# microsoft/ctsTraffic

Hardware: AMD Instinct MI355X
Metric: GiB/s verified, 64 KiB buffers device-resident; % MI355X HBM roofline (higher is better)
Workload: dtype u8

## Files before the change

ctstraffic_amd/csrc/cts_engine.cpp:

```cpp
#include <hip/hip_runtime_api.h>

#include <algorithm>
#include <atomic>
#include <cctype>
#include <chrono>
#include <condition_variable>
#include <cstdio>
#include <cstdlib>
#include <cstring>
#include <memory>
#include <mutex>
#include <new>
#include <string>
#include <system_error>
#include <thread>
#include <vector>

#include "cts_engine.h"
#include "cts_internal.hpp"
#include "cts_slices.hpp"

struct Mailbox;

struct cts_engine {
// ... 440 lines not shown
    if (parts == nullptr && slots == nullptr) return;
    DeviceQuiesce q(e->device);
    if (parts) (void)hipHostFree(parts);
    if (slots) (void)hipHostFree(slots);
}

const cts::LaunchGeometry& cts::engine_geometry(const cts_engine* e, int* device)
{
    if (device != nullptr) *device = e->device;
    return e->geo;
}

extern "C" {

const char* cts_version(void) { return "ctstraffic_amd 0.3.0 (gfx950)"; }

const char* cts_status_string(int status)
{
    switch (status) {
    case CTS_OK: return "ok";
    case CTS_E_INVALID: return "invalid argument";
    case CTS_E_HIP: return "HIP runtime error";
    case CTS_E_NOMEM: return "out of memory";
    case CTS_E_NO_DEVICE: return "no such HIP device";
    case CTS_E_UNAVAILABLE: return "runtime library unavailable (RCCL)";
    case CTS_E_TIMEOUT: return "timed out (nothing freed; retry)";
    default: return "unknown status";
    }
}

int cts_engine_create(int device, cts_engine** out)
{
    if (out == nullptr) return CTS_E_INVALID;
    *out = nullptr;
    int count = 0;
    if (hipGetDeviceCount(&count) != hipSuccess || count <= 0) return CTS_E_NO_DEVICE;
    if (device < 0 || device >= count) return CTS_E_NO_DEVICE;
    DeviceGuard g(device);
    if (!g.ok) return CTS_E_HIP;
    cts_engine* e = new (std::nothrow) cts_engine();
    if (e == nullptr) return CTS_E_NOMEM;
    e->device = device;
    int cus = 0;
    if (hipDeviceGetAttribute(&cus, hipDeviceAttributeMultiprocessorCount, device) == hipSuccess && cus > 0)
        e->geo.num_cus = cus;
    e->geo.blocks_per_cu = env_int("CTS_BLOCKS_PER_CU", e->geo.blocks_per_cu);
    e->geo.nontemporal = env_int("CTS_NT_LOADS", e->geo.nontemporal);
    e->geo.small_threshold = env_int("CTS_SMALL_THRESHOLD", e->geo.small_threshold);
    e->geo.small_blocks_per_cu = env_int("CTS_SMALL_BLOCKS_PER_CU", e->geo.small_blocks_per_cu);
    e->geo.fill_blocks_per_cu = env_int("CTS_FILL_BLOCKS_PER_CU", e->geo.fill_blocks_per_cu);
    e->geo.small_chunk = env_int("CTS_SMALL_CHUNK", e->geo.small_chunk);
    e->geo.fill_nt = env_int("CTS_FILL_NT", e->geo.fill_nt);
    e->geo.ring_fill_blocks_per_cu = env_int("CTS_RING_FILL_BLOCKS_PER_CU", e->geo.ring_fill_blocks_per_cu);
    e->sync_mailbox = env_int("CTS_SYNC_MAILBOX", e->sync_mailbox) ? 1 : 0;
    if (hipStreamCreateWithFlags(&e->stream, hipStreamNonBlocking) != hipSuccess) {
        delete e;
        return CTS_E_HIP;
    }
    void* p = nullptr;
    if (host_alloc_mapped(cts::kSliceMax * sizeof(cts_buf_desc), &p) != CTS_OK) {
        cts_engine_destroy(e);
        return CTS_E_NOMEM;
    }
    e->stage_desc = static_cast<cts_buf_desc*>(p);
    if (host_alloc_mapped(cts::kSliceMax * sizeof(cts_verify_result), &p) != CTS_OK) {
        cts_engine_destroy(e);
        return CTS_E_NOMEM;
    }
    e->stage_res = static_cast<cts_verify_result*>(p);
    *out = e;
    return CTS_OK;
}

int cts_engine_destroy(cts_engine* e)
{
    if (e == nullptr) return CTS_E_INVALID;
    e->mail.reset();
    {
        DeviceGuard g(e->device);
        if (e->stream) {
            (void)hipStreamSynchronize(e->stream);
            (void)hipStreamDestroy(e->stream);
        }
    }
    {
        DeviceQuiesce q(e->device);
        for (auto& st : e->stage_pool) (void)hipHostFree(st.p);
        e->stage_pool.clear();
        if (e->stage) (void)hipHostFree(e->stage);
        if (e->stage_desc) (void)hipHostFree(e->stage_desc);
        if (e->stage_res) (void)hipHostFree(e->stage_res);
        if (e->batch_desc) (void)hipHostFree(e->batch_desc);
        if (e->batch_res) (void)hipHostFree(e->batch_res);
        if (e->batch_ctr) (void)hipHostFree(e->batch_ctr);
    }
    delete e;
    return CTS_OK;
}

int cts_engine_device(const cts_engine* e) { return e ? e->device : CTS_E_INVALID; }

int cts_engine_numa_node(const cts_engine* e)
{
    if (e == nullptr) return -1;
    char bus[64] = {0};
    if (hipDeviceGetPCIBusId(bus, (int)sizeof(bus), e->device) != hipSuccess) return -1;
// ... 507 lines not shown
```

ctstraffic_amd/csrc/cts_internal.hpp:

```cpp
#pragma once

#include <hip/hip_runtime_api.h>
#include <stdint.h>

#include "cts_connections.h"
#include "cts_engine.h"
#include "cts_media_stream.h"
#include "cts_media_stream_conns.h"

namespace cts {

constexpr int kCounterSlots = 8;
enum CounterSlot {
    kBytesChecked = 0,
    kBytesOk = 1,
    kBuffersChecked = 2,
    kBuffersFailed = 3,
    kMismatchedBytes = 4,
    kConnectionsFailed = 5
};
constexpr int kCounterCount = 6;
static_assert(kCounterCount <= kCounterSlots, "counters fit a shard line");

inline cts_counters_ex counters_ex_of(const uint64_t* v)
{
    return cts_counters_ex{v[kBytesChecked],  v[kBytesOk],         v[kBuffersChecked],
                           v[kBuffersFailed], v[kMismatchedBytes], v[kConnectionsFailed]};
}
inline cts_counters counters_of(const cts_counters_ex& x)
{
    return cts_counters{x.bytes_checked, x.bytes_ok, x.buffers_checked, x.buffers_failed, x.mismatched_bytes};
}

constexpr int kVerifyKernelId = 25;
constexpr int kSmallKernelId = 15;
constexpr int kMediaStreamKernelId = 3;

struct LaunchGeometry {
    int num_cus = 256;
    int blocks_per_cu = 4;
    int small_blocks_per_cu = 64;
    int nontemporal = 1;
    int small_threshold = 8192;
    int small_chunk = 0;
    int fill_nt = 2;
    int fill_blocks_per_cu = 1;
    int ring_fill_blocks_per_cu = 4;
};

struct alignas(64) MailSlot {
    uint64_t ptr_exp;
    uint64_t len_seq;
    uint64_t pad[6];
};
static_assert(sizeof(MailSlot) == 64, "one cache line per slot");
inline void mail_write(MailSlot* s, uint64_t ptr_exp, uint64_t len_seq)
{
    __atomic_store_n(&s->ptr_exp, ptr_exp, __ATOMIC_RELAXED);
    __atomic_store_n(&s->len_seq, len_seq, __ATOMIC_RELEASE);
}
struct alignas(16) MailPart {
    uint64_t g0;
    uint64_t g1;
};
constexpr uint32_t kMailPieceBytes = 4096;
#ifndef CTS_MAIL_GROUP
#define CTS_MAIL_GROUP 4
#endif
constexpr uint32_t kMailGroup = CTS_MAIL_GROUP;
#if defined(__HIP__)
__host__ __device__
#endif
inline uint32_t mail_parts(uint64_t ptr, uint32_t len)
{
    if (len == 0) return kMailGroup;
    const uint64_t pieces = (((ptr & 15u) + (uint64_t)len + 15u) / 16u * 16u + kMailPieceBytes - 1) / kMailPieceBytes;
    return pieces < kMailGroup ? (uint32_t)pieces : kMailGroup;
}
constexpr uint32_t kMailMaxGroups = 64;
constexpr uint32_t kMailSkip = 0xFFFFFFFFu;
struct MailStarts {
    uint64_t j[kMailMaxGroups];
};
hipError_t launch_mailbox(const MailSlot* slots, MailPart* parts, uint32_t per_group, const MailStarts& starts,
                          uint32_t groups, uint64_t idle_ticks, hipStream_t stream, uint64_t delay_ticks = 0);

hipError_t launch_counters_fold(const void* block, uint64_t* out, bool accumulate, hipStream_t stream);

hipError_t launch_verify(const uint8_t* arena, uint64_t arena_bytes, const cts_buf_desc* descs, uint32_t n,
                         uint32_t max_length_hint, cts_verify_result* results, uint64_t* counters,
                         uint32_t* conn_first_fail, uint32_t n_conns, hipStream_t stream,
                         const LaunchGeometry& geo);

hipError_t launch_verify_strided(const uint8_t* arena, uint64_t arena_bytes, uint32_t stride, const uint32_t* lens,
                                 uint32_t n, uint32_t skip_head, uint32_t expected, uint32_t conn_index,
                                 cts_verify_result* results, uint64_t* counters, uint32_t* conn_first_fail,
                                 uint32_t n_conns, hipStream_t stream, const LaunchGeometry& geo);

hipError_t launch_verify_at(const uint8_t* arena, uint64_t arena_bytes, const cts_buf_desc* descs, uint32_t n,
                            uint32_t max_length_hint, cts_verify_result* results, uint64_t* counters,
                            uint32_t* conn_first_fail, uint32_t n_conns, uint32_t base_index, hipStream_t stream,
// ... 80 lines not shown
```

ctstraffic_amd/csrc/cts_kernels.hip:

```cpp
#include <hip/hip_runtime.h>

#include <type_traits>

#include "cts_internal.hpp"

namespace cts {

typedef uint32_t u32x4 __attribute__((ext_vector_type(4)));
constexpr uint32_t kNone = 0xFFFFFFFFu;
constexpr int kBlock = 256;

__device__ __forceinline__ uint32_t pattern_byte_dev(uint32_t pos)
{
    pos &= 0xFFFFu;
    return (pos & 1u) ? (pos >> 9) : ((pos >> 1) & 0xFFu);
}

__device__ __forceinline__ u32x4 expected_chunk(uint32_t q, uint32_t sh)
{
    const uint32_t k = q >> 1;
    const uint32_t base = __umul24(k, 0x10001u) + 0x10000u;
    const uint32_t w0 = base & 0x7FFF7FFFu;
    const uint32_t w1 = (base + 0x20002u) & 0x7FFF7FFFu;
    const uint32_t w2 = (base + 0x40004u) & 0x7FFF7FFFu;
    const uint32_t w3 = (base + 0x60006u) & 0x7FFF7FFFu;
    const uint32_t w4 = (base + 0x80008u) & 0x7FFF7FFFu;
    return u32x4{__builtin_amdgcn_alignbyte(w1, w0, sh), __builtin_amdgcn_alignbyte(w2, w1, sh),
                 __builtin_amdgcn_alignbyte(w3, w2, sh), __builtin_amdgcn_alignbyte(w4, w3, sh)};
}

__device__ __forceinline__ uint32_t nonzero_bytes(uint32_t x)
{
    return (((x & 0x7F7F7F7Fu) + 0x7F7F7F7Fu) | x) & 0x80808080u;
}

__device__ __forceinline__ uint32_t low_bytes_mask(int nb)
{
    return (uint32_t)((1ull << (8 * nb)) - 1ull);
}

__device__ __forceinline__ u32x4 range_mask(uint32_t lo, uint32_t hi)
{
    u32x4 m;
#pragma unroll
    for (int w = 0; w < 4; ++w) {
        int a = (int)lo - 4 * w;
        int b = (int)hi - 4 * w;
        a = a < 0 ? 0 : (a > 4 ? 4 : a);
        b = b < 0 ? 0 : (b > 4 ? 4 : b);
        m[w] = (b > a) ? (low_bytes_mask(b) & ~low_bytes_mask(a)) : 0u;
    }
    return m;
}

// ... 875 lines not shown
    }
    uint64_t v[kCounterCount];
    v[kRefBytesRecv] = wave_sum64(bytes_recv);
    v[kRefBytesOk] = wave_sum64(bytes_ok);
    v[kRefBuffersRecv] = wave_sum(bufs_recv);
    v[kRefBuffersFailed] = wave_sum(bufs_failed);
    v[kRefBytesAfterFailure] = wave_sum64(bytes_after);
    v[kRefBuffersAfterFailure] = wave_sum(bufs_after);
    if ((threadIdx.x & 63u) == 0u) {
#pragma unroll
        for (int k = 0; k < kCounterCount; ++k) red[threadIdx.x / 64][k] = v[k];
    }
    __syncthreads();
    if (threadIdx.x < (unsigned)kCounterCount) {
        uint64_t sum = 0;
#pragma unroll
        for (int w = 0; w < kBlock / 64; ++w) sum += red[w][threadIdx.x];
        if (sum)
            atomicAdd((unsigned long long*)&ref[(blockIdx.x % CTS_COUNTER_SHARDS) * kCounterSlots + threadIdx.x],
                      (unsigned long long)sum);
    }
}


__device__ __forceinline__ void block_add_six(const uint64_t (&v)[kCounterCount], uint64_t (*red)[kCounterCount],
                                              uint64_t* __restrict__ block)
{
    if ((threadIdx.x & 63u) == 0u) {
#pragma unroll
        for (int k = 0; k < kCounterCount; ++k) red[threadIdx.x / 64][k] = v[k];
    }
    __syncthreads();
    if (threadIdx.x < (unsigned)kCounterCount) {
        uint64_t sum = 0;
#pragma unroll
        for (int w = 0; w < kBlock / 64; ++w) sum += red[w][threadIdx.x];
        if (sum)
            atomicAdd((unsigned long long*)&block[(blockIdx.x % CTS_COUNTER_SHARDS) * kCounterSlots + threadIdx.x],
                      (unsigned long long)sum);
    }
}

__device__ __forceinline__ void conn_run_add(cts_conn_state* __restrict__ state, uint32_t conn, uint32_t n_conns,
                                             uint64_t recv, uint64_t after, uint32_t nrecv, uint32_t nafter)
{
    if (conn >= n_conns) return;
    unsigned long long* p = reinterpret_cast<unsigned long long*>(state + conn);
    if (recv) atomicAdd(p + 0, (unsigned long long)recv);
    if (nrecv) atomicAdd(p + 1, (unsigned long long)nrecv);
    if (after) atomicAdd(p + 2, (unsigned long long)after);
    if (nafter) atomicAdd(p + 3, (unsigned long long)nafter);
}

template <bool NT, bool STRIDED>
__global__ void __launch_bounds__(kBlock)
    conn_accumulate(uint64_t arena_bytes, VSource src, uint32_t n, uint32_t base_index,
                    const uint32_t* __restrict__ conn_first_fail, uint32_t n_conns, uint64_t* __restrict__ ref,
                    cts_conn_state* __restrict__ state, uint32_t span)
{
    __shared__ uint64_t red[kBlock / 64][kCounterCount];
    const uint32_t lane = threadIdx.x & 63u;
    const uint64_t lo = ((uint64_t)blockIdx.x * (kBlock / 64) + threadIdx.x / 64) * span;
    const uint64_t hi = lo + span < (uint64_t)n ? lo + span : (uint64_t)n;
    uint64_t bytes_recv = 0, bytes_ok = 0, bytes_after = 0;
    uint32_t bufs_recv = 0, bufs_failed = 0, bufs_after = 0;
    __shared__ uint64_t tail_sum[kBlock / 64][4];
    __shared__ uint32_t tail_key[kBlock / 64][2];
    uint32_t ckey = kNone, cnrecv = 0, cnafter = 0;
    uint64_t crecv = 0, cafter = 0;
    bool whole = true;
    uint64_t pa = 0, pb = 0;
    uint32_t pnrecv = 0, pnafter = 0;
    bool parked = false;
    uint32_t ring_first = kNone;
    if constexpr (STRIDED) ring_first = src.conn_index < n_conns ? conn_first_fail[src.conn_index] : kNone;
    cts_buf_desc dn = cts_buf_desc{0, 0, 65536u, 0, 0};
    if (lo < hi) dn = refview_desc<NT, STRIDED>(src, lo + lane < hi ? lo + lane : hi - 1);
    for (uint64_t t = lo; t < hi; t += 64) {
        const uint64_t i = t + lane;
        const cts_buf_desc d = dn;
        if (t + 64 < hi) dn = refview_desc<NT, STRIDED>(src, i + 64 < hi ? i + 64 : hi - 1);
        const bool ok = i < hi && !desc_bad(d, arena_bytes);
        const uint32_t key = ok ? d.conn_index : kNone;
        const uint32_t first = STRIDED ? ring_first : (key < n_conns ? conn_first_fail[key] : kNone);
        const uint32_t g = base_index + (uint32_t)i;
        const uint32_t vlen = ok ? d.length - d.skip_head : 0u;
        const bool recv = ok && g <= first, after = ok && g > first;
        if (recv) {
            bytes_recv += vlen;
            bufs_recv += 1u;
            if (g < first) bytes_ok += vlen;
            else bufs_failed += 1u;
        } else if (after) {
            bytes_after += vlen;
            bufs_after += 1u;
        }
        const uint32_t below = (uint32_t)__shfl_up((int)key, 1, 64);
        const bool head = lane == 0u || key != below;
        const uint64_t heads = __ballot(head);
        const uint32_t h = 63u - (uint32_t)__builtin_clzll(heads & (~0ull >> (63u - lane)));
        const bool merge = (uint32_t)__shfl((int)key, 0, 64) == ckey;
        if (heads == 1ull && merge) {
            pa += recv ? vlen : 0u;
            pb += after ? vlen : 0u;
            pnrecv += recv ? 1u : 0u;
            pnafter += after ? 1u : 0u;
            parked = true;
            continue;
        }
        if (parked) {
            crecv += wave_sum64(pa);
            cafter += wave_sum64(pb);
            cnrecv += wave_sum(pnrecv);
            cnafter += wave_sum(pnafter);
            pa = pb = 0;
            pnrecv = pnafter = 0;
            parked = false;
        }
        uint64_t a = recv ? vlen : 0u, b = after ? vlen : 0u;
        uint32_t c = (recv ? 1u : 0u) | (after ? 0x10000u : 0u);
#pragma unroll
        for (uint32_t off = 1; off < 64u; off <<= 1) {
            const uint64_t ua = (uint64_t)__shfl_up((unsigned long long)a, off, 64);
            const uint64_t ub = (uint64_t)__shfl_up((unsigned long long)b, off, 64);
            const uint32_t uc = (uint32_t)__shfl_up((int)c, off, 64);
            if (lane >= h + off) {
                a += ua;
                b += ub;
                c += uc;
            }
        }
        uint32_t nrecv = c & 0xFFFFu, nafter = c >> 16;
        whole = whole && heads == 1ull && (merge || t == lo);
        if (merge && h == 0u) {
            a += crecv;
            b += cafter;
            nrecv += cnrecv;
            nafter += cnafter;
        }
        if (!merge && lane == 0u) conn_run_add(state, ckey, n_conns, crecv, cafter, cnrecv, cnafter);
        const bool tail = lane == 63u || ((heads >> (lane + 1u)) & 1ull) != 0ull;
        if (tail && lane != 63u) conn_run_add(state, key, n_conns, a, b, nrecv, nafter);
        ckey = (uint32_t)__shfl((int)key, 63, 64);
        crecv = (uint64_t)__shfl((unsigned long long)a, 63, 64);
        cafter = (uint64_t)__shfl((unsigned long long)b, 63, 64);
        cnrecv = (uint32_t)__shfl((int)nrecv, 63, 64);
        cnafter = (uint32_t)__shfl((int)nafter, 63, 64);
    }
    if (parked) {
        crecv += wave_sum64(pa);
        cafter += wave_sum64(pb);
        cnrecv += wave_sum(pnrecv);
        cnafter += wave_sum(pnafter);
    }
    if (lane == 0u) {
        tail_sum[threadIdx.x / 64][0] = crecv;
        tail_sum[threadIdx.x / 64][1] = cafter;
        tail_sum[threadIdx.x / 64][2] = cnrecv;
        tail_sum[threadIdx.x / 64][3] = cnafter;
        tail_key[threadIdx.x / 64][0] = ckey;
        tail_key[threadIdx.x / 64][1] = whole ? 1u : 0u;
    }
    __syncthreads();
    if (threadIdx.x == 0u) {
        uint32_t key = tail_key[0][0];
        uint64_t acc[4] = {tail_sum[0][0], tail_sum[0][1], tail_sum[0][2], tail_sum[0][3]};
        for (int w = 1; w < kBlock / 64; ++w) {
            if (tail_key[w][1] == 0u || tail_key[w][0] != key) {
                conn_run_add(state, key, n_conns, acc[0], acc[1], (uint32_t)acc[2], (uint32_t)acc[3]);
                key = tail_key[w][0];
                acc[0] = acc[1] = acc[2] = acc[3] = 0;
            }
#pragma unroll
            for (int k = 0; k < 4; ++k) acc[k] += tail_sum[w][k];
        }
        conn_run_add(state, key, n_conns, acc[0], acc[1], (uint32_t)acc[2], (uint32_t)acc[3]);
    }
    uint64_t v[kCounterCount];
    v[kRefBytesRecv] = wave_sum64(bytes_recv);
    v[kRefBytesOk] = wave_sum64(bytes_ok);
    v[kRefBuffersRecv] = wave_sum(bufs_recv);
    v[kRefBuffersFailed] = wave_sum(bufs_failed);
    v[kRefBytesAfterFailure] = wave_sum64(bytes_after);
    v[kRefBuffersAfterFailure] = wave_sum(bufs_after);
    block_add_six(v, red, ref);
}

enum CloseSlot {
    kCloseClosed = 0,
    kCloseSuccessful = 1,
    kCloseDataErrors = 2,
    kCloseNotAllData = 3,
    kCloseTooMuchData = 4,
    kCloseBytesRecv = 5
};
static_assert(kCloseBytesRecv + 1 == kCounterCount, "a close block folds like a counter block");

template <bool NT>
__global__ void __launch_bounds__(kBlock)
    conn_close(const uint32_t* __restrict__ ids, const uint64_t* __restrict__ expected, uint32_t n,
               uint32_t* __restrict__ conn_first_fail, cts_conn_state* __restrict__ state, uint32_t n_conns,
               cts_conn_result* __restrict__ results, uint64_t* __restrict__ block)
{
    __shared__ uint64_t red[kBlock / 64][kCounterCount];
    uint32_t closed = 0, successful = 0, data_errors = 0, not_all = 0, too_much = 0;
    uint64_t bytes = 0;
    const uint64_t step = (uint64_t)gridDim.x * kBlock;
    for (uint64_t i = (uint64_t)blockIdx.x * kBlock + threadIdx.x; i < n; i += step) {
        const uint32_t c = NT ? __builtin_nontemporal_load(ids + i) : ids[i];
        cts_conn_result r = cts_conn_result{0, 0, 0, 0, 0u, 0u, c, 0u};
        if (c >= n_conns) {
            r.flags = CTS_CONN_RESULT_FLAG_BAD_CONN;
        } else {
            const uint32_t first = conn_first_fail[c];
            const cts_conn_state s = state[c];
            uint32_t status = 0u;
            if (first != kNone) {
                status = CTS_STATUS_ERROR_DATA_DID_NOT_MATCH_BIT_PATTERN;
                data_errors += 1u;
            } else if (expected != nullptr) {
                const uint64_t want = NT ? __builtin_nontemporal_load(expected + i) : expected[i];
                if (s.bytes_recv > want) {
                    status = CTS_STATUS_ERROR_TOO_MUCH_DATA_TRANSFERRED;
                    too_much += 1u;
                } else if (s.bytes_recv < want) {
                    status = CTS_STATUS_ERROR_NOT_ALL_DATA_TRANSFERRED;
                    not_all += 1u;
                }
            }
            if (status == 0u) successful += 1u;
            closed += 1u;
            bytes += s.bytes_recv;
            r.bytes_recv = s.bytes_recv;
            r.buffers_recv = s.buffers_recv;
            r.bytes_after_failure = s.bytes_after_failure;
            r.buffers_after_failure = s.buffers_after_failure;
            r.first_fail = first;
            r.status = status;
// ... 13 lines not shown
}

__global__ void __launch_bounds__(kBlock) conn_slots_rebase(uint32_t* __restrict__ conn_first_fail, uint32_t n_conns,
                                                            uint32_t delta)
{
    const uint64_t step = (uint64_t)gridDim.x * kBlock;
    for (uint64_t i = (uint64_t)blockIdx.x * kBlock + threadIdx.x; i < n_conns; i += step) {
        const uint32_t first = conn_first_fail[i];
        if (first != kNone) conn_first_fail[i] = first < delta ? 0u : first - delta;
    }
}

enum UdpSlot {
    kUdpBits = 0,
    kUdpSuccessful = 1,
    kUdpDropped = 2,
    kUdpDuplicate = 3,
    kUdpErrorFrames = 4,
    kUdpDatagrams = 5
};
static_assert(kUdpDatagrams + 1 == kCounterCount, "a UDP block folds like a counter block");

struct MsMeta {
    uint32_t conn;
    int64_t seq;
    uint32_t completed;
    uint32_t fkp;
};

template <bool NT>
__device__ __forceinline__ MsMeta ms_meta(const cts_buf_desc* __restrict__ descs,
                                          const cts_datagram_status* __restrict__ status, uint64_t i)
{
    const uint64_t* dp = reinterpret_cast<const uint64_t*>(descs + i) + 2;
    const uint64_t* sp = reinterpret_cast<const uint64_t*>(status + i);
    const uint64_t c = NT ? __builtin_nontemporal_load(dp) : dp[0];
    const uint64_t a = NT ? __builtin_nontemporal_load(sp) : sp[0];
    const uint64_t b = NT ? __builtin_nontemporal_load(sp + 1) : sp[1];
    return MsMeta{(uint32_t)c, (int64_t)a, (uint32_t)b, (uint32_t)(b >> 32)};
}

__device__ __forceinline__ void ms_run_add(cts_ms_conn_state* state, uint32_t conn, uint32_t n_conns, uint64_t bits,
                                           uint32_t dg, uint32_t after, uint32_t err, uint32_t in)
{
    if (conn >= n_conns) return;
    cts_ms_conn_state* e = state + conn;
    if (bits) atomicAdd((unsigned long long*)&e->bits_received, (unsigned long long)bits);
    if (err) atomicAdd((unsigned long long*)&e->error_frames, (unsigned long long)err);
    if (dg) atomicAdd((unsigned long long*)&e->datagrams, (unsigned long long)dg);
    if (after) atomicAdd((unsigned long long*)&e->datagrams_after_end, (unsigned long long)after);
    if (in) e->received_any = 1u;
}

template <bool NT>
__global__ void __launch_bounds__(kBlock)
    ms_conn_accumulate(const cts_buf_desc* __restrict__ descs, const cts_datagram_status* __restrict__ status,
                       uint32_t n, uint32_t base_index, const uint32_t* __restrict__ conn_first_fail,
                       cts_ms_conn_state* state, uint64_t* __restrict__ frame_bytes, uint64_t frame_elems,
                       uint32_t n_conns, uint64_t* __restrict__ udp, uint32_t span)
{
    __shared__ uint64_t red[kBlock / 64][kCounterCount];
    __shared__ uint64_t tail_sum[kBlock / 64][5];
    __shared__ uint32_t tail_key[kBlock / 64][2];
    const uint32_t lane = threadIdx.x & 63u;
    const uint64_t lo = ((uint64_t)blockIdx.x * (kBlock / 64) + threadIdx.x / 64) * span;
    const uint64_t hi = lo + span < (uint64_t)n ? lo + span : (uint64_t)n;
    uint64_t node_bits = 0;
    uint32_t node_err = 0, node_dg = 0;
    uint32_t ckey = kNone, cdg = 0, cafter = 0, cerr = 0, cin = 0;
    uint64_t cbits = 0;
    bool whole = true;
    uint64_t pbits = 0;
    uint32_t pdg = 0, pafter = 0, perr = 0, pin = 0;
    bool parked = false;
    MsMeta mn = MsMeta{kNone, 0, 0u, 0u};
    if (lo < hi) mn = ms_meta<NT>(descs, status, lo + lane < hi ? lo + lane : hi - 1);
    for (uint64_t t = lo; t < hi; t += 64) {
        const uint64_t i = t + lane;
        const MsMeta m = mn;
        if (t + 64 < hi) mn = ms_meta<NT>(descs, status, i + 64 < hi ? i + 64 : hi - 1);
        const bool ok = i < hi;
        const uint32_t key = ok ? m.conn : kNone;
        const bool has = ok && m.conn < n_conns;
        uint32_t first = kNone, fin = 0u, frames = 0u;
        int64_t head = 0, final_frame = 0;
        uint64_t fbase = 0;
        if (has) {
            const cts_ms_conn_state* e = state + m.conn;
            first = conn_first_fail[m.conn];
            fin = e->finished;
            head = e->head_sequence_number;
            final_frame = e->final_frame;
            fbase = e->frame_base;
            frames = e->frames;
        }
        const uint32_t kind = (m.fkp >> 16) & 0xFFu;
        const bool clean = kind == CTS_DGRAM_DATA && (m.fkp >> 24) != 0u;
        const uint32_t g = base_index + (uint32_t)i;
        uint64_t bits = 0;
        uint32_t dg = 0, after = 0, err = 0, in = 0;
        if (ok) {
            if (has && (fin != 0u || g > first)) {
                after = 1u;
            } else {
                dg = 1u;
                if (has && g == first) {
                    cts_ms_conn_state* e = state + m.conn;
                    e->last_error = kind == CTS_DGRAM_DATA ? CTS_STATUS_ERROR_DATA_DID_NOT_MATCH_BIT_PATTERN
                                                           : CTS_STATUS_ERROR_NOT_ALL_DATA_TRANSFERRED;
                    e->has_failure = 1u;
                } else if (clean) {
                    bits = (uint64_t)m.completed * 8u;
                    if (has) {
                        const bool inside = m.seq <= final_frame && m.seq >= head &&
                                            (uint64_t)(m.seq - head) < (uint64_t)frames;
                        const uint64_t at = inside ? fbase + (uint64_t)(m.seq - 1) % frames : frame_elems;
                        if (at < frame_elems) {
                            atomicAdd((unsigned long long*)&frame_bytes[at], (unsigned long long)m.completed);
                            in = 1u;
                        } else {
                            err = 1u;
                        }
                    }
                }
            }
        }
        node_bits += bits;
        node_err += err;
        node_dg += dg;
        const uint32_t below = (uint32_t)__shfl_up((int)key, 1, 64);
        const bool rhead = lane == 0u || key != below;
        const uint64_t heads = __ballot(rhead);
        const uint32_t h = 63u - (uint32_t)__builtin_clzll(heads & (~0ull >> (63u - lane)));
        const bool merge = (uint32_t)__shfl((int)key, 0, 64) == ckey;
        if (heads == 1ull && merge) {
            pbits += bits;
            pdg += dg;
            pafter += after;
            perr += err;
            pin += in;
            parked = true;
            continue;
        }
        if (parked) {
            cbits += wave_sum64(pbits);
            cdg += wave_sum(pdg);
            cafter += wave_sum(pafter);
            cerr += wave_sum(perr);
            cin += wave_sum(pin);
            pbits = 0;
            pdg = pafter = perr = pin = 0;
            parked = false;
        }
        uint64_t a = bits;
        uint32_t c = dg | (after << 8) | (err << 16) | (in << 24);
#pragma unroll
        for (uint32_t off = 1; off < 64u; off <<= 1) {
            const uint64_t ua = (uint64_t)__shfl_up((unsigned long long)a, off, 64);
            const uint32_t uc = (uint32_t)__shfl_up((int)c, off, 64);
            if (lane >= h + off) {
                a += ua;
                c += uc;
            }
        }
        uint32_t rdg = c & 0xFFu, rafter = (c >> 8) & 0xFFu, rerr = (c >> 16) & 0xFFu, rin = c >> 24;
        whole = whole && heads == 1ull && (merge || t == lo);
        if (merge && h == 0u) {
            a += cbits;
            rdg += cdg;
            rafter += cafter;
            rerr += cerr;
            rin += cin;
        }
        if (!merge && lane == 0u) ms_run_add(state, ckey, n_conns, cbits, cdg, cafter, cerr, cin);
        const bool tail = lane == 63u || ((heads >> (lane + 1u)) & 1ull) != 0ull;
        if (tail && lane != 63u) ms_run_add(state, key, n_conns, a, rdg, rafter, rerr, rin);
        ckey = (uint32_t)__shfl((int)key, 63, 64);
        cbits = (uint64_t)__shfl((unsigned long long)a, 63, 64);
        cdg = (uint32_t)__shfl((int)rdg, 63, 64);
        cafter = (uint32_t)__shfl((int)rafter, 63, 64);
        cerr = (uint32_t)__shfl((int)rerr, 63, 64);
        cin = (uint32_t)__shfl((int)rin, 63, 64);
    }
    if (parked) {
        cbits += wave_sum64(pbits);
        cdg += wave_sum(pdg);
        cafter += wave_sum(pafter);
        cerr += wave_sum(perr);
        cin += wave_sum(pin);
    }
    if (lane == 0u) {
        tail_sum[threadIdx.x / 64][0] = cbits;
        tail_sum[threadIdx.x / 64][1] = cdg;
        tail_sum[threadIdx.x / 64][2] = cafter;
        tail_sum[threadIdx.x / 64][3] = cerr;
        tail_sum[threadIdx.x / 64][4] = cin;
        tail_key[threadIdx.x / 64][0] = ckey;
        tail_key[threadIdx.x / 64][1] = whole ? 1u : 0u;
    }
    __syncthreads();
    if (threadIdx.x == 0u) {
        uint32_t key = tail_key[0][0];
        uint64_t acc[5] = {tail_sum[0][0], tail_sum[0][1], tail_sum[0][2], tail_sum[0][3], tail_sum[0][4]};
        for (int w = 1; w < kBlock / 64; ++w) {
            if (tail_key[w][1] == 0u || tail_key[w][0] != key) {
                ms_run_add(state, key, n_conns, acc[0], (uint32_t)acc[1], (uint32_t)acc[2], (uint32_t)acc[3],
                           (uint32_t)acc[4]);
                key = tail_key[w][0];
                acc[0] = acc[1] = acc[2] = acc[3] = acc[4] = 0;
            }
#pragma unroll
            for (int k = 0; k < 5; ++k) acc[k] += tail_sum[w][k];
        }
        ms_run_add(state, key, n_conns, acc[0], (uint32_t)acc[1], (uint32_t)acc[2], (uint32_t)acc[3], (uint32_t)acc[4]);
    }
    uint64_t v[kCounterCount] = {0, 0, 0, 0, 0, 0};
    v[kUdpBits] = wave_sum64(node_bits);
    v[kUdpErrorFrames] = wave_sum(node_err);
    v[kUdpDatagrams] = wave_sum(node_dg);
    block_add_six(v, red, udp);
}

__global__ void __launch_bounds__(kBlock)
    ms_conn_render(const uint32_t* __restrict__ ids, uint32_t n, cts_ms_conn_state* state,
                   uint64_t* __restrict__ frame_bytes, uint32_t n_conns, uint64_t* __restrict__ udp,
                   uint32_t* __restrict__ codes)
{
    __shared__ uint64_t red[kBlock / 64][kCounterCount];
    uint32_t successful = 0, duplicate = 0;
    uint64_t dropped = 0;
    const uint64_t step = (uint64_t)gridDim.x * kBlock;
    for (uint64_t i = (uint64_t)blockIdx.x * kBlock + threadIdx.x; i < n; i += step) {
        const uint32_t c = ids[i];
        uint32_t code = 0u;
        if (c < n_conns) {
            cts_ms_conn_state* e = state + c;
            if (e->last_error != CTS_STATUS_IO_RUNNING || e->frames == 0u) {
                code = e->finished;
            } else {
                const uint32_t wheel = e->timer_wheel_offset + 1u;
                e->timer_wheel_offset = wheel;
                int64_t head = e->head_sequence_number;
                const int64_t final_frame = e->final_frame;
                if (wheel >= e->initial_buffer_frames && head <= final_frame) {
                    if (e->received_any == 0u && head == 1) {
                        e->dropped_frames += (uint64_t)final_frame;
                        dropped += (uint64_t)final_frame;
                        e->finished = CTS_MS_CONN_FATAL;
                        e->last_error = CTS_STATUS_ERROR_NOT_ALL_DATA_TRANSFERRED;
                        code = 2u;
                    } else {
                        uint64_t* slot = frame_bytes + e->frame_base + (uint64_t)(head - 1) % e->frames;
                        const uint64_t got = *slot;
                        if (got == (uint64_t)e->frame_size_bytes) {
                            e->successful_frames += 1u;
                            successful += 1u;
                        } else if (got < (uint64_t)e->frame_size_bytes) {
                            e->dropped_frames += 1u;
                            dropped += 1u;
                        } else {
                            e->duplicate_frames += 1u;
                            duplicate += 1u;
                        }
                        *slot = 0;
                        head += 1;
                        e->head_sequence_number = head;
                    }
                }
                if (code == 0u && head > final_frame) {
                    e->finished = CTS_MS_CONN_FINISHED;
                    e->last_error = 0u;
                    code = 1u;
                }
// ... 1045 lines not shown
        verify_quad_kernel<true, true><<<cg.grid, kBlock, 0, stream>>>(arena, arena_bytes, src, n, results, counters,
                                                                       conn_first_fail, n_conns, cg.per, base_index);
    else
        verify_quad_kernel<false, true><<<cg.grid, kBlock, 0, stream>>>(arena, arena_bytes, src, n, results, counters,
                                                                        conn_first_fail, n_conns, cg.per, base_index);
    return hipGetLastError();
}

hipError_t launch_verify_strided(const uint8_t* arena, uint64_t arena_bytes, uint32_t stride, const uint32_t* lens,
                                 uint32_t n, uint32_t skip_head, uint32_t expected, uint32_t conn_index,
                                 cts_verify_result* results, uint64_t* counters, uint32_t* conn_first_fail,
                                 uint32_t n_conns, hipStream_t stream, const LaunchGeometry& geo)
{
    return launch_verify_strided_at(arena, arena_bytes, stride, lens, n, skip_head, expected, conn_index, results,
                                    counters, conn_first_fail, n_conns, 0u, stream, geo);
}

constexpr int kRefviewBlocksPerCu = 8;
template <bool STRIDED>
static hipError_t launch_refview_src(uint64_t arena_bytes, const VSource& src, uint32_t n, uint32_t base_index,
                                     const uint32_t* conn_first_fail, uint32_t n_conns, uint64_t* ref_counters,
                                     hipStream_t stream, const LaunchGeometry& geo)
{
    if (n == 0) return hipSuccess;
    const uint64_t want = ((uint64_t)n + kBlock - 1) / kBlock;
    const uint64_t cap = (uint64_t)(geo.num_cus > 0 ? geo.num_cus : 1) * kRefviewBlocksPerCu;
    const uint32_t grid = (uint32_t)(want < cap ? want : cap);
    if (geo.nontemporal)
        refview_accumulate<true, STRIDED><<<grid, kBlock, 0, stream>>>(arena_bytes, src, n, base_index, conn_first_fail,
                                                                       n_conns, ref_counters);
    else
        refview_accumulate<false, STRIDED><<<grid, kBlock, 0, stream>>>(arena_bytes, src, n, base_index, conn_first_fail,
                                                                        n_conns, ref_counters);
    return hipGetLastError();
}

hipError_t launch_refview(uint64_t arena_bytes, const cts_buf_desc* descs, uint32_t n, uint32_t base_index,
                          const uint32_t* conn_first_fail, uint32_t n_conns, uint64_t* ref_counters, hipStream_t stream,
                          const LaunchGeometry& geo)
{
    return launch_refview_src<false>(arena_bytes, VSource{descs, nullptr, 0u, 0u, 0u, 0u}, n, base_index,
                                     conn_first_fail, n_conns, ref_counters, stream, geo);
}

hipError_t launch_refview_strided(uint64_t arena_bytes, uint32_t stride, const uint32_t* lens, uint32_t n,
                                  uint32_t skip_head, uint32_t conn_index, uint32_t base_index,
                                  const uint32_t* conn_first_fail, uint32_t n_conns, uint64_t* ref_counters,
                                  hipStream_t stream, const LaunchGeometry& geo)
{
    return launch_refview_src<true>(arena_bytes, VSource{nullptr, lens, stride, skip_head, 0u, conn_index}, n,
                                    base_index, conn_first_fail, n_conns, ref_counters, stream, geo);
}

template <bool STRIDED>
static hipError_t launch_conn_accumulate_src(uint64_t arena_bytes, const VSource& src, uint32_t n, uint32_t base_index,
                                             const uint32_t* conn_first_fail, uint32_t n_conns, uint64_t* ref_counters,
                                             cts_conn_state* conn_state, hipStream_t stream, const LaunchGeometry& geo)
{
    if (n == 0) return hipSuccess;
    const uint64_t want = ((uint64_t)n + kBlock - 1) / kBlock;
    const uint64_t cap = (uint64_t)(geo.num_cus > 0 ? geo.num_cus : 1) * kRefviewBlocksPerCu;
    const uint32_t grid = (uint32_t)(want < cap ? want : cap);
    const uint64_t waves = (uint64_t)grid * (kBlock / 64);
    const uint32_t span = (uint32_t)((((uint64_t)n + waves - 1) / waves + 63u) / 64u * 64u);
    if (geo.nontemporal)
        conn_accumulate<true, STRIDED><<<grid, kBlock, 0, stream>>>(arena_bytes, src, n, base_index, conn_first_fail,
                                                                    n_conns, ref_counters, conn_state, span);
    else
        conn_accumulate<false, STRIDED><<<grid, kBlock, 0, stream>>>(arena_bytes, src, n, base_index, conn_first_fail,
                                                                     n_conns, ref_counters, conn_state, span);
    return hipGetLastError();
}

hipError_t launch_conn_accumulate(uint64_t arena_bytes, const cts_buf_desc* descs, uint32_t n, uint32_t base_index,
                                  const uint32_t* conn_first_fail, uint32_t n_conns, uint64_t* ref_counters,
                                  cts_conn_state* conn_state, hipStream_t stream, const LaunchGeometry& geo)
{
    return launch_conn_accumulate_src<false>(arena_bytes, VSource{descs, nullptr, 0u, 0u, 0u, 0u}, n, base_index,
                                             conn_first_fail, n_conns, ref_counters, conn_state, stream, geo);
}

hipError_t launch_conn_accumulate_strided(uint64_t arena_bytes, uint32_t stride, const uint32_t* lens, uint32_t n,
                                          uint32_t skip_head, uint32_t conn_index, uint32_t base_index,
                                          const uint32_t* conn_first_fail, uint32_t n_conns, uint64_t* ref_counters,
                                          cts_conn_state* conn_state, hipStream_t stream, const LaunchGeometry& geo)
{
    return launch_conn_accumulate_src<true>(arena_bytes, VSource{nullptr, lens, stride, skip_head, 0u, conn_index}, n,
                                            base_index, conn_first_fail, n_conns, ref_counters, conn_state, stream,
                                            geo);
}

static inline uint32_t lane_per_item_grid(uint32_t n, const LaunchGeometry& geo)
{
    const uint64_t want = ((uint64_t)n + kBlock - 1) / kBlock;
    const uint64_t cap = (uint64_t)(geo.num_cus > 0 ? geo.num_cus : 1) * kRefviewBlocksPerCu;
    return (uint32_t)(want < cap ? want : cap);
}

hipError_t launch_conn_close(const uint32_t* conn_ids, const uint64_t* expected_bytes, uint32_t n,
                             uint32_t* conn_first_fail, cts_conn_state* conn_state, uint32_t n_conns,
                             cts_conn_result* results, uint64_t* close_counters, hipStream_t stream,
                             const LaunchGeometry& geo)
{
    if (n == 0) return hipSuccess;
    const uint32_t grid = lane_per_item_grid(n, geo);
    if (geo.nontemporal)
        conn_close<true><<<grid, kBlock, 0, stream>>>(conn_ids, expected_bytes, n, conn_first_fail, conn_state, n_conns,
                                                      results, close_counters);
    else
        conn_close<false><<<grid, kBlock, 0, stream>>>(conn_ids, expected_bytes, n, conn_first_fail, conn_state,
                                                       n_conns, results, close_counters);
    return hipGetLastError();
}

hipError_t launch_conn_slots_rebase(uint32_t* conn_first_fail, uint32_t n_conns, uint32_t delta, hipStream_t stream,
                                    const LaunchGeometry& geo)
{
    if (n_conns == 0 || delta == 0) return hipSuccess;
    conn_slots_rebase<<<lane_per_item_grid(n_conns, geo), kBlock, 0, stream>>>(conn_first_fail, n_conns, delta);
    return hipGetLastError();
}

hipError_t launch_ms_conn_accumulate(const cts_buf_desc* descs, const cts_datagram_status* status, uint32_t n,
                                     uint32_t base_index, const uint32_t* conn_first_fail, cts_ms_conn_state* conns,
                                     uint64_t* frame_bytes, uint64_t frame_elems, uint32_t n_conns,
                                     uint64_t* udp_counters, hipStream_t stream, const LaunchGeometry& geo)
{
    if (n == 0) return hipSuccess;
    const uint32_t grid = lane_per_item_grid(n, geo);
    const uint64_t waves = (uint64_t)grid * (kBlock / 64);
    const uint32_t span = (uint32_t)((((uint64_t)n + waves - 1) / waves + 63u) / 64u * 64u);
    if (geo.nontemporal)
        ms_conn_accumulate<true><<<grid, kBlock, 0, stream>>>(descs, status, n, base_index, conn_first_fail, conns,
                                                              frame_bytes, frame_elems, n_conns, udp_counters, span);
    else
        ms_conn_accumulate<false><<<grid, kBlock, 0, stream>>>(descs, status, n, base_index, conn_first_fail, conns,
                                                               frame_bytes, frame_elems, n_conns, udp_counters, span);
    return hipGetLastError();
}

hipError_t launch_ms_conn_render(const uint32_t* conn_ids, uint32_t n, cts_ms_conn_state* conns, uint64_t* frame_bytes,
                                 uint32_t n_conns, uint64_t* udp_counters, uint32_t* codes, hipStream_t stream,
                                 const LaunchGeometry& geo)
{
    if (n == 0) return hipSuccess;
    ms_conn_render<<<lane_per_item_grid(n, geo), kBlock, 0, stream>>>(conn_ids, n, conns, frame_bytes, n_conns,
                                                                      udp_counters, codes);
    return hipGetLastError();
}

hipError_t launch_ms_conn_close(const uint32_t* conn_ids, uint32_t n, uint32_t* conn_first_fail,
                                cts_ms_conn_state* conns, uint64_t* frame_bytes, uint32_t n_conns,
                                cts_ms_conn_result* results, uint64_t* close_counters, hipStream_t stream,
                                const LaunchGeometry& geo)
{
    if (n == 0) return hipSuccess;
    const uint64_t want = ((uint64_t)n + kBlock / 64 - 1) / (kBlock / 64);
    const uint64_t cap = (uint64_t)(geo.num_cus > 0 ? geo.num_cus : 1) * kRefviewBlocksPerCu;
    ms_conn_close<<<(uint32_t)(want < cap ? want : cap), kBlock, 0, stream>>>(conn_ids, n, conn_first_fail, conns,
                                                                             frame_bytes, n_conns, results,
                                                                             close_counters);
    return hipGetLastError();
}

static inline uint32_t batched_fill_grid(uint32_t n, const LaunchGeometry& geo)
{
    const uint64_t cap = (uint64_t)geo.num_cus * (uint64_t)(geo.ring_fill_blocks_per_cu > 0 ? geo.ring_fill_blocks_per_cu : 4);
    const uint64_t want = ((uint64_t)n + kFillBatch - 1) / kFillBatch;
    return (uint32_t)(want < cap ? want : cap);
}

hipError_t launch_fill(uint8_t* arena, uint64_t arena_bytes, const cts_buf_desc* descs, uint32_t n,
                       uint32_t max_length_hint, hipStream_t stream, const LaunchGeometry& geo)
{
    if (n == 0) return hipSuccess;
    const bool small = max_length_hint != 0 && max_length_hint <= (uint32_t)geo.small_threshold;
    const bool nts = geo.fill_nt == 2 ? small : geo.fill_nt != 0;
    const uint32_t sgrid = grid_for(n, kBlock / 64, geo), lgrid = grid_for(n, 1, geo, geo.fill_blocks_per_cu);
    if (!small && max_length_hint != 0) {
        const uint32_t ppb = (uint32_t)(((uint64_t)max_length_hint + kFillPiece - 1) / kFillPiece);
        const uint64_t total = (uint64_t)n * ppb;
        const uint64_t cap = (uint64_t)geo.num_cus * (uint64_t)(geo.fill_blocks_per_cu > 0 ? geo.fill_blocks_per_cu : 1);
        const uint32_t pgrid = (uint32_t)(total < cap ? total : cap);
        if (nts) fill_pieces_kernel<true><<<pgrid, kBlock, 0, stream>>>(arena, arena_bytes, descs, n, ppb);
        else fill_pieces_kernel<false><<<pgrid, kBlock, 0, stream>>>(arena, arena_bytes, descs, n, ppb);
        return hipGetLastError();
    }
    if (nts) {
        if (small) fill_kernel<64, true><<<sgrid, kBlock, 0, stream>>>(arena, arena_bytes, descs, n);
        else fill_kernel<kBlock, true><<<lgrid, kBlock, 0, stream>>>(arena, arena_bytes, descs, n);
// ... 159 lines not shown
```

Baseline: 6654.

## Aggregate per-connection counters in an LDS hash table before global atomics

Adds a block-local open-addressing hash table in shared memory that collects per-connection run totals in conn_accumulate (non-strided) and ms_conn_accumulate, then flushes each slot once to global state. The goal is fewer global atomics on hot connection entries. The grid is now sized by a new conn_blocks_per_cu knob, and dynamic LDS is raised when needed. The cost is the table clear and flush work, lower occupancy from the LDS use, and a fallback to global atomics when probing fails.

```diff
diff --git a/ctstraffic_amd/csrc/cts_engine.cpp b/ctstraffic_amd/csrc/cts_engine.cpp
--- a/ctstraffic_amd/csrc/cts_engine.cpp
+++ b/ctstraffic_amd/csrc/cts_engine.cpp
@@ -516,6 +516,9 @@
     e->geo.small_chunk = env_int("CTS_SMALL_CHUNK", e->geo.small_chunk);
     e->geo.fill_nt = env_int("CTS_FILL_NT", e->geo.fill_nt);
     e->geo.ring_fill_blocks_per_cu = env_int("CTS_RING_FILL_BLOCKS_PER_CU", e->geo.ring_fill_blocks_per_cu);
+    e->geo.conn_table_slots =
+        cts::conn_table_slots_clamped(env_int("CTS_CONN_TABLE_SLOTS", e->geo.conn_table_slots));
+    e->geo.conn_blocks_per_cu = env_int("CTS_CONN_BLOCKS_PER_CU", e->geo.conn_blocks_per_cu);
     e->sync_mailbox = env_int("CTS_SYNC_MAILBOX", e->sync_mailbox) ? 1 : 0;
     if (hipStreamCreateWithFlags(&e->stream, hipStreamNonBlocking) != hipSuccess) {
         delete e;
diff --git a/ctstraffic_amd/csrc/cts_internal.hpp b/ctstraffic_amd/csrc/cts_internal.hpp
--- a/ctstraffic_amd/csrc/cts_internal.hpp
+++ b/ctstraffic_amd/csrc/cts_internal.hpp
@@ -46,7 +46,17 @@
     int fill_nt = 2;
     int fill_blocks_per_cu = 1;
     int ring_fill_blocks_per_cu = 4;
+    int conn_table_slots = 1024;
+    int conn_blocks_per_cu = 4;
 };
+
+inline int conn_table_slots_clamped(int requested)
+{
+    if (requested <= 0) return 0;
+    int slots = 16;
+    while (slots < 4096 && slots * 2 <= requested) slots *= 2;
+    return slots;
+}
 
 struct alignas(64) MailSlot {
     uint64_t ptr_exp;
diff --git a/ctstraffic_amd/csrc/cts_kernels.hip b/ctstraffic_amd/csrc/cts_kernels.hip
--- a/ctstraffic_amd/csrc/cts_kernels.hip
+++ b/ctstraffic_amd/csrc/cts_kernels.hip
@@ -1,5 +1,6 @@
 #include <hip/hip_runtime.h>
 
+#include <atomic>
 #include <type_traits>
 
 #include "cts_internal.hpp"
@@ -981,12 +982,90 @@
     if (nafter) atomicAdd(p + 3, (unsigned long long)nafter);
 }
 
+constexpr uint32_t kConnTableProbes = 4;
+constexpr uint32_t kConnTableSlotBytes = 4u * 8u + 4u;
+
+__host__ __device__ __forceinline__ uint32_t conn_slots_of(uint32_t span_slots)
+{
+    const uint32_t k = span_slots & 63u;
+    return k != 0u ? 8u << k : 0u;
+}
+static inline uint32_t conn_span_slots(uint32_t span, uint32_t slots)
+{
+    uint32_t k = 0;
+    while (slots != 0u && (8u << k) < slots) ++k;
+    return span | k;
+}
+extern __shared__ unsigned long long conn_table_lds[];
+
+__device__ __forceinline__ uint32_t* conn_table_keys(uint32_t slots)
+{
+    return reinterpret_cast<uint32_t*>(conn_table_lds + 4u * (size_t)slots);
+}
+
+__device__ __forceinline__ void conn_table_clear(uint32_t slots)
+{
+    if (slots == 0u) return;
+    uint32_t* keys = conn_table_keys(slots);
+    for (uint32_t s = threadIdx.x; s < 4u * slots; s += kBlock) conn_table_lds[s] = 0ull;
+    for (uint32_t s = threadIdx.x; s < slots; s += kBlock) keys[s] = kNone;
+    __syncthreads();
+}
+
+__device__ __forceinline__ uint32_t conn_table_claim(uint32_t slots, uint32_t key)
+{
+    uint32_t* keys = conn_table_keys(slots);
+    const uint32_t mask = slots - 1u;
+    uint32_t s = (key ^ (key >> (31u - (uint32_t)__builtin_clz(slots)))) & mask;
+    for (uint32_t p = 0; p < kConnTableProbes; ++p) {
+        const uint32_t old = atomicCAS(&keys[s], kNone, key);
+        if (old == kNone || old == key) return s;
+        s = (s + 1u) & mask;
+    }
+    return kNone;
+}
+
+__device__ __forceinline__ bool conn_table_add(uint32_t slots, uint32_t conn, uint64_t v0, uint64_t v1, uint64_t v2,
+                                               uint64_t v3)
+{
+    if (slots == 0u) return false;
+    const uint32_t s = conn_table_claim(slots, conn);
+    if (s == kNone) return false;
+    if (v0) atomicAdd(&conn_table_lds[s], (unsigned long long)v0);
+    if (v1) atomicAdd(&conn_table_lds[slots + s], (unsigned long long)v1);
+    if (v2) atomicAdd(&conn_table_lds[2u * slots + s], (unsigned long long)v2);
+    if (v3) atomicAdd(&conn_table_lds[3u * slots + s], (unsigned long long)v3);
+    return true;
+}
+
+__device__ __forceinline__ void conn_run_book(uint32_t slots, cts_conn_state* __restrict__ state, uint32_t conn,
+                                              uint32_t n_conns, uint64_t recv, uint64_t after, uint32_t nrecv,
+                                              uint32_t nafter)
+{
+    if (conn >= n_conns) return;
+    if (!conn_table_add(slots, conn, recv, nrecv, after, nafter))
+        conn_run_add(state, conn, n_conns, recv, after, nrecv, nafter);
+}
+
+__device__ __forceinline__ void conn_table_flush(uint32_t slots, cts_conn_state* __restrict__ state, uint32_t n_conns)
+{
+    const uint32_t* keys = conn_table_keys(slots);
+    for (uint32_t s = threadIdx.x; s < slots; s += kBlock) {
+        const uint32_t key = keys[s];
+        if (key != kNone)
+            conn_run_add(state, key, n_conns, conn_table_lds[s], conn_table_lds[2u * slots + s],
+                         (uint32_t)conn_table_lds[slots + s], (uint32_t)conn_table_lds[3u * slots + s]);
+    }
+}
+
 template <bool NT, bool STRIDED>
 __global__ void __launch_bounds__(kBlock)
     conn_accumulate(uint64_t arena_bytes, VSource src, uint32_t n, uint32_t base_index,
                     const uint32_t* __restrict__ conn_first_fail, uint32_t n_conns, uint64_t* __restrict__ ref,
-                    cts_conn_state* __restrict__ state, uint32_t span)
-{
+                    cts_conn_state* __restrict__ state, uint32_t span_slots)
+{
+    const uint32_t span = span_slots & ~63u;
+    const uint32_t tslots = STRIDED ? 0u : conn_slots_of(span_slots);
     __shared__ uint64_t red[kBlock / 64][kCounterCount];
     const uint32_t lane = threadIdx.x & 63u;
     const uint64_t lo = ((uint64_t)blockIdx.x * (kBlock / 64) + threadIdx.x / 64) * span;
@@ -1005,6 +1084,7 @@
     if constexpr (STRIDED) ring_first = src.conn_index < n_conns ? conn_first_fail[src.conn_index] : kNone;
     cts_buf_desc dn = cts_buf_desc{0, 0, 65536u, 0, 0};
     if (lo < hi) dn = refview_desc<NT, STRIDED>(src, lo + lane < hi ? lo + lane : hi - 1);
+    conn_table_clear(tslots);
     for (uint64_t t = lo; t < hi; t += 64) {
         const uint64_t i = t + lane;
         const cts_buf_desc d = dn;
@@ -1067,9 +1147,9 @@
             nrecv += cnrecv;
             nafter += cnafter;
         }
-        if (!merge && lane == 0u) conn_run_add(state, ckey, n_conns, crecv, cafter, cnrecv, cnafter);
+        if (!merge && lane == 0u) conn_run_book(tslots, state, ckey, n_conns, crecv, cafter, cnrecv, cnafter);
         const bool tail = lane == 63u || ((heads >> (lane + 1u)) & 1ull) != 0ull;
-        if (tail && lane != 63u) conn_run_add(state, key, n_conns, a, b, nrecv, nafter);
+        if (tail && lane != 63u) conn_run_book(tslots, state, key, n_conns, a, b, nrecv, nafter);
         ckey = (uint32_t)__shfl((int)key, 63, 64);
         crecv = (uint64_t)__shfl((unsigned long long)a, 63, 64);
         cafter = (uint64_t)__shfl((unsigned long long)b, 63, 64);
@@ -1096,14 +1176,14 @@
         uint64_t acc[4] = {tail_sum[0][0], tail_sum[0][1], tail_sum[0][2], tail_sum[0][3]};
         for (int w = 1; w < kBlock / 64; ++w) {
             if (tail_key[w][1] == 0u || tail_key[w][0] != key) {
-                conn_run_add(state, key, n_conns, acc[0], acc[1], (uint32_t)acc[2], (uint32_t)acc[3]);
+                conn_run_book(tslots, state, key, n_conns, acc[0], acc[1], (uint32_t)acc[2], (uint32_t)acc[3]);
                 key = tail_key[w][0];
                 acc[0] = acc[1] = acc[2] = acc[3] = 0;
             }
 #pragma unroll
             for (int k = 0; k < 4; ++k) acc[k] += tail_sum[w][k];
         }
-        conn_run_add(state, key, n_conns, acc[0], acc[1], (uint32_t)acc[2], (uint32_t)acc[3]);
+        conn_run_book(tslots, state, key, n_conns, acc[0], acc[1], (uint32_t)acc[2], (uint32_t)acc[3]);
     }
     uint64_t v[kCounterCount];
     v[kRefBytesRecv] = wave_sum64(bytes_recv);
@@ -1113,6 +1193,7 @@
     v[kRefBytesAfterFailure] = wave_sum64(bytes_after);
     v[kRefBuffersAfterFailure] = wave_sum(bufs_after);
     block_add_six(v, red, ref);
+    if (tslots) conn_table_flush(tslots, state, n_conns);
 }
 
 enum CloseSlot {
@@ -1232,13 +1313,34 @@
     if (in) e->received_any = 1u;
 }
 
+__device__ __forceinline__ void ms_run_book(uint32_t slots, cts_ms_conn_state* state, uint32_t conn, uint32_t n_conns,
+                                            uint64_t bits, uint32_t dg, uint32_t after, uint32_t err, uint32_t in)
+{
+    if (conn >= n_conns) return;
+    if (!conn_table_add(slots, conn, bits, err, dg, (uint64_t)after | ((uint64_t)in << 32)))
+        ms_run_add(state, conn, n_conns, bits, dg, after, err, in);
+}
+
+__device__ __forceinline__ void ms_table_flush(uint32_t slots, cts_ms_conn_state* state, uint32_t n_conns)
+{
+    const uint32_t* keys = conn_table_keys(slots);
+    for (uint32_t s = threadIdx.x; s < slots; s += kBlock) {
+        const uint32_t key = keys[s];
+        if (key == kNone) continue;
+        const uint64_t ai = conn_table_lds[3u * slots + s];
+        ms_run_add(state, key, n_conns, conn_table_lds[s], (uint32_t)conn_table_lds[2u * slots + s], (uint32_t)ai,
+                   (uint32_t)conn_table_lds[slots + s], (uint32_t)(ai >> 32));
+    }
+}
+
 template <bool NT>
 __global__ void __launch_bounds__(kBlock)
     ms_conn_accumulate(const cts_buf_desc* __restrict__ descs, const cts_datagram_status* __restrict__ status,
                        uint32_t n, uint32_t base_index, const uint32_t* __restrict__ conn_first_fail,
                        cts_ms_conn_state* state, uint64_t* __restrict__ frame_bytes, uint64_t frame_elems,
-                       uint32_t n_conns, uint64_t* __restrict__ udp, uint32_t span)
-{
+                       uint32_t n_conns, uint64_t* __restrict__ udp, uint32_t span_slots)
+{
+    const uint32_t span = span_slots & ~63u, slots = conn_slots_of(span_slots);
     __shared__ uint64_t red[kBlock / 64][kCounterCount];
     __shared__ uint64_t tail_sum[kBlock / 64][5];
     __shared__ uint32_t tail_key[kBlock / 64][2];
@@ -1255,6 +1357,7 @@
     bool parked = false;
     MsMeta mn = MsMeta{kNone, 0, 0u, 0u};
     if (lo < hi) mn = ms_meta<NT>(descs, status, lo + lane < hi ? lo + lane : hi - 1);
+    conn_table_clear(slots);
     for (uint64_t t = lo; t < hi; t += 64) {
         const uint64_t i = t + lane;
         const MsMeta m = mn;
@@ -1352,9 +1455,9 @@
             rerr += cerr;
             rin += cin;
         }
-        if (!merge && lane == 0u) ms_run_add(state, ckey, n_conns, cbits, cdg, cafter, cerr, cin);
+        if (!merge && lane == 0u) ms_run_book(slots, state, ckey, n_conns, cbits, cdg, cafter, cerr, cin);
         const bool tail = lane == 63u || ((heads >> (lane + 1u)) & 1ull) != 0ull;
-        if (tail && lane != 63u) ms_run_add(state, key, n_conns, a, rdg, rafter, rerr, rin);
+        if (tail && lane != 63u) ms_run_book(slots, state, key, n_conns, a, rdg, rafter, rerr, rin);
         ckey = (uint32_t)__shfl((int)key, 63, 64);
         cbits = (uint64_t)__shfl((unsigned long long)a, 63, 64);
         cdg = (uint32_t)__shfl((int)rdg, 63, 64);
@@ -1384,7 +1487,7 @@
         uint64_t acc[5] = {tail_sum[0][0], tail_sum[0][1], tail_sum[0][2], tail_sum[0][3], tail_sum[0][4]};
         for (int w = 1; w < kBlock / 64; ++w) {
             if (tail_key[w][1] == 0u || tail_key[w][0] != key) {
-                ms_run_add(state, key, n_conns, acc[0], (uint32_t)acc[1], (uint32_t)acc[2], (uint32_t)acc[3],
+                ms_run_book(slots, state, key, n_conns, acc[0], (uint32_t)acc[1], (uint32_t)acc[2], (uint32_t)acc[3],
                            (uint32_t)acc[4]);
                 key = tail_key[w][0];
                 acc[0] = acc[1] = acc[2] = acc[3] = acc[4] = 0;
@@ -1392,13 +1495,14 @@
 #pragma unroll
             for (int k = 0; k < 5; ++k) acc[k] += tail_sum[w][k];
         }
-        ms_run_add(state, key, n_conns, acc[0], (uint32_t)acc[1], (uint32_t)acc[2], (uint32_t)acc[3], (uint32_t)acc[4]);
+        ms_run_book(slots, state, key, n_conns, acc[0], (uint32_t)acc[1], (uint32_t)acc[2], (uint32_t)acc[3], (uint32_t)acc[4]);
     }
     uint64_t v[kCounterCount] = {0, 0, 0, 0, 0, 0};
     v[kUdpBits] = wave_sum64(node_bits);
     v[kUdpErrorFrames] = wave_sum(node_err);
     v[kUdpDatagrams] = wave_sum(node_dg);
     block_add_six(v, red, udp);
+    if (slots) ms_table_flush(slots, state, n_conns);
 }
 
 __global__ void __launch_bounds__(kBlock)
@@ -2550,23 +2654,58 @@
                                     base_index, conn_first_fail, n_conns, ref_counters, stream, geo);
 }
 
+struct ConnGrid {
+    uint32_t grid, span, slots;
+    size_t lds;
+};
+static inline ConnGrid conn_grid(uint32_t n, const LaunchGeometry& geo, bool table)
+{
+    uint32_t slots = table ? (uint32_t)conn_table_slots_clamped(geo.conn_table_slots) : 0u;
+    const int bpc = slots != 0u && geo.conn_blocks_per_cu > 0 ? geo.conn_blocks_per_cu : kRefviewBlocksPerCu;
+    const uint64_t want = ((uint64_t)n + kBlock - 1) / kBlock;
+    const uint64_t cap = (uint64_t)(geo.num_cus > 0 ? geo.num_cus : 1) * (uint64_t)bpc;
+    const uint32_t grid = (uint32_t)(want < cap ? want : cap);
+    const uint64_t waves = (uint64_t)grid * (kBlock / 64);
+    const uint32_t span = (uint32_t)((((uint64_t)n + waves - 1) / waves + 63u) / 64u * 64u);
+    while (slots > 16u && (uint64_t)slots >= 4u * (uint64_t)span * (kBlock / 64)) slots /= 2u;
+    return ConnGrid{grid, span, slots, (size_t)slots * kConnTableSlotBytes};
+}
+
+template <auto Kernel>
+static hipError_t conn_table_lds_limit(size_t lds)
+{
+    const auto kernel = Kernel;
+    static std::atomic<uint64_t> raised{0};
+    if (lds <= 64u * 1024u) return hipSuccess;
+    int device = 0;
+    hipError_t err = hipGetDevice(&device);
+    if (err != hipSuccess) return err;
+    const uint64_t bit = device < 64 ? 1ull << device : 0ull;
+    if (bit != 0ull && (raised.load(std::memory_order_relaxed) & bit) != 0ull) return hipSuccess;
+    err = hipFuncSetAttribute(reinterpret_cast<const void*>(kernel), hipFuncAttributeMaxDynamicSharedMemorySize,
+                              160 * 1024 - 2048);
+    if (err == hipSuccess) raised.fetch_or(bit, std::memory_order_relaxed);
+    return err;
+}
+
 template <bool STRIDED>
 static hipError_t launch_conn_accumulate_src(uint64_t arena_bytes, const VSource& src, uint32_t n, uint32_t base_index,
                                              const uint32_t* conn_first_fail, uint32_t n_conns, uint64_t* ref_counters,
                                              cts_conn_state* conn_state, hipStream_t stream, const LaunchGeometry& geo)
 {
     if (n == 0) return hipSuccess;
-    const uint64_t want = ((uint64_t)n + kBlock - 1) / kBlock;
-    const uint64_t cap = (uint64_t)(geo.num_cus > 0 ? geo.num_cus : 1) * kRefviewBlocksPerCu;
-    const uint32_t grid = (uint32_t)(want < cap ? want : cap);
-    const uint64_t waves = (uint64_t)grid * (kBlock / 64);
-    const uint32_t span = (uint32_t)((((uint64_t)n + waves - 1) / waves + 63u) / 64u * 64u);
+    const ConnGrid cg = conn_grid(n, geo, !STRIDED);
+    const hipError_t err = geo.nontemporal ? conn_table_lds_limit<conn_accumulate<true, STRIDED>>(cg.lds)
+                                           : conn_table_lds_limit<conn_accumulate<false, STRIDED>>(cg.lds);
+    if (err != hipSuccess) return err;
     if (geo.nontemporal)
-        conn_accumulate<true, STRIDED><<<grid, kBlock, 0, stream>>>(arena_bytes, src, n, base_index, conn_first_fail,
-                                                                    n_conns, ref_counters, conn_state, span);
+        conn_accumulate<true, STRIDED><<<cg.grid, kBlock, cg.lds, stream>>>(
+            arena_bytes, src, n, base_index, conn_first_fail, n_conns, ref_counters, conn_state,
+            conn_span_slots(cg.span, cg.slots));
     else
-        conn_accumulate<false, STRIDED><<<grid, kBlock, 0, stream>>>(arena_bytes, src, n, base_index, conn_first_fail,
-                                                                     n_conns, ref_counters, conn_state, span);
+        conn_accumulate<false, STRIDED><<<cg.grid, kBlock, cg.lds, stream>>>(
+            arena_bytes, src, n, base_index, conn_first_fail, n_conns, ref_counters, conn_state,
+            conn_span_slots(cg.span, cg.slots));
     return hipGetLastError();
 }
 
@@ -2625,15 +2764,20 @@
                                      uint64_t* udp_counters, hipStream_t stream, const LaunchGeometry& geo)
 {
     if (n == 0) return hipSuccess;
-    const uint32_t grid = lane_per_item_grid(n, geo);
-    const uint64_t waves = (uint64_t)grid * (kBlock / 64);
-    const uint32_t span = (uint32_t)((((uint64_t)n + waves - 1) / waves + 63u) / 64u * 64u);
+    const ConnGrid cg = conn_grid(n, geo, true);
+    const hipError_t err = geo.nontemporal ? conn_table_lds_limit<ms_conn_accumulate<true>>(cg.lds)
+                                           : conn_table_lds_limit<ms_conn_accumulate<false>>(cg.lds);
+    if (err != hipSuccess) return err;
     if (geo.nontemporal)
-        ms_conn_accumulate<true><<<grid, kBlock, 0, stream>>>(descs, status, n, base_index, conn_first_fail, conns,
-                                                              frame_bytes, frame_elems, n_conns, udp_counters, span);
+        ms_conn_accumulate<true><<<cg.grid, kBlock, cg.lds, stream>>>(descs, status, n, base_index, conn_first_fail,
+                                                                      conns, frame_bytes, frame_elems, n_conns,
+                                                                      udp_counters,
+                                                                      conn_span_slots(cg.span, cg.slots));
     else
-        ms_conn_accumulate<false><<<grid, kBlock, 0, stream>>>(descs, status, n, base_index, conn_first_fail, conns,
-                                                               frame_bytes, frame_elems, n_conns, udp_counters, span);
+        ms_conn_accumulate<false><<<cg.grid, kBlock, cg.lds, stream>>>(descs, status, n, base_index, conn_first_fail,
+                                                                       conns, frame_bytes, frame_elems, n_conns,
+                                                                       udp_counters,
+                                                                      conn_span_slots(cg.span, cg.slots));
     return hipGetLastError();
 }
 
```

New measurement: 6626. About the same (-0.4%).
